# vivansxu/rafiki

Hardware: AMD Instinct MI355X
Metric: images/sec aggregate over concurrent VGG-small 32x32x3 HPO trials (1 trial/GPU) (higher is better)
Workload: dtype fp32; 1 GPU; model=VGG-small 32x32x3 (8 conv3x3+BN+ReLU, 4 maxpool, FC512, FC10), global_batch=256, per_trial_batch=256, parallelism=single trial, 1 GPU, optimizer=SGD nesterov momentum + wd (fused flat-arena kernel), hipgraph=True

## Files before the change

### rafiki_amd/engine/convnet.py

```python
from __future__ import annotations

import math
import os
import warnings
from typing import List, Optional, Sequence

import numpy as np
import torch
import torch.nn.functional as TF

from ..ops import f32 as S
from ..ops import functional as F
from ..ops.graphs import capture as _capture, device_sync as _device_sync
from .flat import FlatAdam, FlatParams, FlatSGD, init_const, init_kaiming

VGG_SMALL_CFG = (64, 64, 'M', 128, 128, 'M', 256, 256, 'M', 512, 512, 'M')
DTYPES = ('fp32', 'bf16')


def default_dtype() -> str:
    d = os.environ.get('RAFIKI_DTYPE', 'fp32').lower()
    d = {'float32': 'fp32', 'f32': 'fp32', 'bfloat16': 'bf16'}.get(d, d)
    if d not in DTYPES:
        raise ValueError('RAFIKI_DTYPE must be one of {}'.format(DTYPES))
# ... 344 lines not shown
                else:
                    d = F.conv_dgrad(dy, fl.wb(name + '.w'))

    def _bn_on_load(self, bi, B, ww):
        if ww is None or bi + 1 >= len(self.blocks):
            return False
        name, cin, cout, pool, hw = self.blocks[bi]
        nxt = self.blocks[bi + 1]
        return (not pool and nxt[1] == cout and nxt[4] == hw and ww.lazy('u4b', bi + 1) is not None
                and S.bn_on_load_ok(B, hw, hw, cout, nxt[2]))

    def _fwd_bwd_gpu_f32(self, x, labels):
        fl = self.flat
        B = x.shape[0]
        accs = self._bn_accumulators()
        if not self._acc_zeroed_by_prologue:
            self._bn_acc_flat.zero_()
        ww = self._wino_train()
        if ww is not None:
            ww.refresh()
        acts, saved, h = [x], [], x
        pros, hpro = [None], None
        for bi, (name, cin, cout, pool, hw) in enumerate(self.blocks):
            wk = ww.conv_sets(bi) if ww is not None else {}
            if not self.bn:
                c = self._block_coeffs(bi)
                y = S.conv_fwd(h, fl.w(name + '.w'), bias=fl.w(name + '.b'),
                               act=F.ACT_NONE if pool else F.ACT_RELU, **wk)
                h = S.bn_eval(y, c[2], c[3], pool=True, act=F.ACT_RELU) if pool else y
                saved.append((y, c))
                acts.append(h)
                continue
            rm, rv = self.running_stats(bi)
            y = S.conv_fwd(h, fl.w(name + '.w'), stats_acc=accs[bi][0], pro=hpro, **wk)
            if self._bn_on_load(bi, B, ww):
                coeffs = S.bn_finalize(y, accs[bi][0], B * hw * hw, fl.w(name + '.gamma'), fl.w(name + '.beta'),
                                       self.bn_eps, rm, rv, self.bn_momentum)
                h, hpro = y, coeffs
            else:
                h, coeffs = S.bn_fwd(y, accs[bi][0], B * hw * hw, fl.w(name + '.gamma'), fl.w(name + '.beta'),
                                     self.bn_eps, rm, rv, self.bn_momentum, pool=pool, act=F.ACT_RELU)
                hpro = None
            saved.append((y, coeffs))
            acts.append(h)
            pros.append(hpro)
        in_saved = None
        if self.input_bn:
            raw = h.reshape(B, 1, 1, self.feat_dim)
            acc_f, acc_b = accs[-1]
            S.col_stats(raw.view(B, self.feat_dim), acc_f)
            rm, rv = self.running_stats('in')
            h, coeffs = S.bn_fwd(raw, acc_f, B, fl.w('in_bn.gamma'), fl.w('in_bn.beta'), self.bn_eps, rm, rv,
                                 self.bn_momentum, pool=False, act=F.ACT_NONE)
            in_saved = (raw, coeffs)
        feat = h.reshape(B, self.feat_dim)
        if self.feature_dropout > 0.0:
            self._drop(feat, -1, self.feature_dropout, forward=True)
        fc_in = [feat]
        z = feat
        for k, (name, di, do, _) in enumerate(self.fcs):
            z = S.linear(z, fl.w(name + '.w'), fl.w(name + '.b'), act=F.ACT_RELU)
            if self.dropout > 0.0:
                self._drop(z, k, self.dropout, forward=True)
            fc_in.append(z)
        dlogits = torch.empty((B, self.ncls_p), dtype=torch.float32, device=self.device)
        k_top = len(self.fcs) - 1
        if self.fused_head and S.head_ok(self.ncls_p, self.d_last):
# ... 26 lines not shown
            else:
                S.softmax_xent(logits, labels, self.num_classes, dlogits=dlogits, loss_sum=self.loss_sum,
                               correct=self.correct, counted=self.seen)
            S.linear_dw(dlogits, fc_in[-1], out=fl.g('out.w'))
            S.colsum(dlogits, fl.g('out.b'))
            d, wname = dlogits, 'out'
        for k in range(k_top, -1, -1):
            name = self.fcs[k][0]
            d = S.linear_dx(d, fl.w(wname + '.w'), gate=fc_in[k + 1])
            if self.dropout > 0.0:
                self._drop(d, k, self.dropout)
            S.linear_dw(d, fc_in[k], out=fl.g(name + '.w'))
            S.colsum(d, fl.g(name + '.b'))
            wname = name
        if not self.blocks and not self.input_bn:
            return
        if wname is not None:
            d = S.linear_dx(d, fl.w(wname + '.w'))
            if self.feature_dropout > 0.0:
                self._drop(d, -1, self.feature_dropout)
        if self.input_bn:
            raw, coeffs = in_saved
            S.bn_bwd(d.view(B, 1, 1, self.feat_dim), raw, coeffs, fl.w('in_bn.gamma'), accs[-1][1], pool=False,
                     act=F.ACT_NONE, dgamma=fl.g('in_bn.gamma'), dbeta=fl.g('in_bn.beta'))
            return
        d = d.view(B, self.feat_hw, self.feat_hw, -1)
        wt = self._conv_wt()
        if wt is not None:
            wt.begin_step()
        reduced = False
        for bi in range(len(self.blocks) - 1, -1, -1):
            name, cin, cout, pool, hw = self.blocks[bi]
            y, coeffs = saved[bi]
            if self.bn:
                dy = S.bn_bwd(d, y, coeffs, fl.w(name + '.gamma'), accs[bi][1], pool=pool, act=F.ACT_RELU,
                              dgamma=fl.g(name + '.gamma'), dbeta=fl.g(name + '.beta'), reduced=reduced)
            else:
                dy = S.bn_bwd(d, y, coeffs, self._ones[:cout], accs[bi][1], pool=pool, act=F.ACT_RELU,
                              dbeta=fl.g(name + '.b'), reduced=reduced, count=float('inf'))
            S.conv_wgrad(dy, acts[bi], out=fl.g(name + '.w').view(cout, -1),
                         xpro=pros[bi] if self.bn else None)
            if bi == 0:
                break
            py, pco = saved[bi - 1]
            pname, pcin, pcout, ppool, phw = self.blocks[bi - 1]
            wl = wt.lazy(bi - 1)
            dk = dict(ww.conv_sets(bi, dgrad=True) if ww is not None else {}, cin=cin)
            if not ppool:
                d = S.conv_dgrad(dy, wl, bnb=(py, pco, accs[bi - 1][1]), **dk)
                reduced = True
            elif phw == 2 * hw and not (hw & (hw - 1)):
                d = S.conv_dgrad(dy, wl, bnp=(py, pco, accs[bi - 1][1]), **dk)
                reduced = True
            else:
                d = S.conv_dgrad(dy, wl, **dk)
                reduced = False
        if ww is not None:
            ww.end_step()

    def _wino_train(self):
        if not (self.f32 and S.WINO and self.blocks and self.device.type == 'cuda'):
            return None
        ww = getattr(self, '_ww', None)
        if ww is None:
            fl = self.flat
            ww = self._ww = S.WinoWeights(fl.master, [fl.w(b[0] + '.w') for b in self.blocks],
# ... 635 lines not shown
```

### rafiki_amd/ops/_lib.py

```python
from __future__ import annotations

import ctypes as C
import os
import threading
from pathlib import Path

_NATIVE = Path(__file__).resolve().parent.parent / "_native"
KERNEL_LIB = Path(os.environ["RAFIKI_KERNEL_LIB"]) if os.environ.get("RAFIKI_KERNEL_LIB") else \
    _NATIVE / "librafiki_kernels.so"

_lock = threading.Lock()
_lib = None

vp, i32, i64, f32, f64 = C.c_void_p, C.c_int, C.c_longlong, C.c_float, C.c_double
u32p = C.POINTER(C.c_uint)

_SIGS = {
    "rk_igemm": [i32, i32, i32, vp, vp, vp, vp, vp, vp, i32, i32, i32, i32, i32, i32, i32, i32, i32, i32,
                 i32, i32, i64, i32, f32, f32, i64, i64, vp],
    "rk_hconv": [i32, i32, vp, vp, vp, vp, vp, vp, i32, i32, i32, i32, i32, i32, i32, i32, f32, f32, i64, i64, i32,
                 vp],
    "rk_hconv_wgrad": [vp, vp, vp, i32, i32, i32, i32, i32, i32, i64, i64, vp],
    "rk_bn_bwd_reduce_acc": [vp, vp, vp, vp, vp, i32, i32, i32, i32, i32, i32, i32, i32, f32, vp],
    "rk_bn_bwd_apply_acc": [vp, vp, vp, vp, i32, f64, vp, vp, vp, vp, i32, vp, i32, i32, i32, i32, i32, i32, f32, vp],
# ... 31 lines not shown
    "rk_nonfinite": [vp, i64, vp, vp],
    "rk_reduce_slabs": [vp, i32, i64, vp, i32, f32, vp],
    "rk_colsum": [vp, i32, i32, i32, vp, i32, vp],
    "rk_ensemble_mean": [vp, i32, i64, vp, vp, vp],
    "rk_cast_f32_bf16": [vp, vp, i64, vp],
    "rk_pack_nhwc": [vp, i32, i32, i32, i32, i32, i32, f32, f32, vp, vp],
    "rk_philox": [vp, i64, i32, i32, f32, f32, C.c_ulonglong, C.c_uint, vp, vp],
    "rk_lrelu_pixelnorm": [vp, vp, vp, i32, i32, f32, f32, vp, vp],
    "rk_mbstd": [i32, vp, vp, vp, i32, i32, i32, i32, i32, i32, vp, vp, vp, vp],
    "rk_colsum_part": [vp, i32, i32, i32, i32, vp, vp],
    "rk_lstm_fwd": [vp, vp, i32, i32, i32, vp, vp, vp, vp],
    "rk_lstm_bwd": [vp, i32, i32, i32, vp, vp, vp, vp, vp],
    "rk_lstm_fwd32": [vp, vp, i32, i32, i32, vp, vp, vp, vp],
    "rk_lstm_bwd32": [vp, i32, i32, i32, vp, vp, vp, vp, vp],
    "rk_wino_weights": [vp, vp, vp, i32, i32, vp],
    "rk_wino_conv_grp": [vp, vp, vp, vp, vp, i32, vp, i32, i32, i32, i32, i32, i32, i32, i32, i64, i64, i64, i64, vp],
    "rk_wino_wgrad": [vp, vp, vp, i32, i32, i32, i32, i32, i32, i32, vp],
    "rk_wino4_weights": [vp, vp, vp, i32, i32, vp],
    "rk_wino4b_weights": [vp, vp, vp, i32, i32, vp],
    "rk_wino4_conv_grp": [vp, vp, vp, vp, vp, i32, vp, i32, i32, i32, i32, i32, i32, i32, i32, i64, i64, i64, i64, vp,
                          vp],
    "rk_wino4_wgrad": [vp, vp, vp, i32, i32, i32, i32, i32, i32, i32, i32, vp, vp],
    "rk_wino4_pt_transform": [vp, vp, vp, vp, i32, i32, i32, i32, i32, vp, vp],
    "rk_wino4_pt_output": [vp, vp, i32, i32, i32, i32, i64, vp],
    "rk_wino4_pt_input": [vp, vp, i32, i32, i32, i32, vp, vp],
    "rk_wino4_pt_conv_out": [vp, vp, vp, vp, i32, vp, i32, i32, i32, i32, i32, i32, i64, i32, f32, vp],
    "rk_wino2s_conv_grp": [vp, vp, vp, vp, vp, i32, vp, i32, i32, i32, i32, i32, i32, i32, i32, i64, i64, i64, i64, vp],
    "rk_sgemm": [i32, i32, i32, vp, vp, vp, vp, vp, i32, vp, i32, i32, i32, i32, i32, i32, i32, i32, i32, i32, i32,
                 i64, i32, f32, f32, i64, i64, vp],
    "rk_bnf_fwd": [vp, vp, i32, f64, vp, vp, f32, vp, vp, f32, vp, vp, vp, vp, i32, i32, i32, i32, i32, i32, f32, vp],
    "rk_bnf_bwd_reduce": [vp, vp, vp, vp, i32, i32, i32, i32, i32, i32, i32, i32, f32, vp],
    "rk_bnf_bwd_apply": [vp, vp, vp, vp, i32, f64, vp, vp, vp, i32, vp, i32, i32, i32, i32, i32, i32, f32, vp],
    "rk_bnf_colstats": [vp, vp, i32, i32, vp, vp],
    "rk_swt": [vp, vp, vp, i32, vp, vp],
    "rk_colsum_f32": [vp, i32, i32, i32, vp, i32, i32, vp],
    "rk_lrelu_gate_f32": [vp, vp, vp, i64, f32, vp],
    "rk_lrelu_gate_colsum_f32": [vp, vp, vp, i32, i32, f32, vp, i32, vp],
    "rk_wgan_loss_fwd": [vp, i32, i32, vp, i32, f32, f32, f32, vp, vp, vp, vp],
    "rk_wgan_mix": [vp, vp, vp, vp, vp, i32, i32, vp],
    "rk_wgan_loss_bwd": [vp, vp, i32, i32, vp, i32, f32, f32, f32, vp, vp, vp, vp],
    "rk_sreduce_epi": [vp, i32, i32, i32, vp, i32, f32, f32, vp, i32, vp, i32, i32, vp],
    "rk_sgemm_grp": [i32, i32, i32, vp, vp, vp, vp] + [i32] * 10 + [i32, i64, i32, f32, f32, i64, i64, i32, i64, i64,
                                                                     i64, i64, vp],
    "rk_bnf_eval_grp": [vp, vp, vp, vp, i32, i32, i32, i32, i32, i32, i32, f32, vp],
    "rk_pack_nhwc_f32": [vp, i32, i32, i32, i32, i32, i32, f32, f32, vp, vp, i32, vp],
    "rk_softmax_xent_f32": [vp, i32, vp, i32, i32, i32, f32, vp, i32, vp, vp, vp, vp, vp],
    "rk_softmax_xent_f32_soft": [vp, i32, vp, vp, vp, f32, i32, i32, i32, f32, vp, i32, vp, vp, vp, vp],
    "rk_sgemm_g": [i32, i32, i32, vp, vp, vp, vp] + [i32] * 14 + [u32p, u32p, C.c_uint, i32, i64, i32, i64, i32, f32,
                                                                 f32, i64, i64, vp],
    "rk_resample2x": [i32, i32, vp, vp, i32, i32, i32, i32, f32, vp],
    "rk_s2t_weights": [vp, vp, i32, i32, vp],
    "rk_box_weights": [i32, vp, vp, i32, i32, f32, vp],
    "rk_wflip_t": [vp, vp, i32, i32, i32, vp],
    "rk_mbstd_f32": [i32, vp, vp, vp, i32, i32, i32, i32, i32, i32, vp, vp, vp, vp],
    "rk_lrelu_pixelnorm_f32": [vp, vp, vp, i32, i32, f32, f32, vp, vp],
    "rk_embedding_fwd": [vp, vp, vp, i32, i32, i32, vp],
    "rk_embedding_bwd": [vp, vp, vp, i32, i32, i32, i32, vp, i64, vp],
    "rk_tag_embed_fwd": [vp, vp, vp, vp, i32, i32, i32, f32, C.c_ulonglong, i32, vp, vp],
    "rk_tag_embed_bwd": [vp, vp, vp, vp, vp, vp, vp, i32, i32, i32, vp],
    "rk_tag_transpose": [vp, vp, i32, i32, i32, vp],
    "rk_tag_add": [vp, vp, vp, i64, vp],
    "rk_softmax_xent_f32s": [vp, i32, vp, i32, i32, i32, vp, vp, i32, vp, vp],
    "rk_head_fwd_bwd": [vp, i32, i32, vp, vp, i32, vp, i32, f32, vp, vp, i32, vp, vp, vp, vp],
    "rk_head_fwd_bwd_soft": [vp, i32, i32, vp, vp, i32, vp, vp, vp, f32, i32, f32, vp, vp, i32, vp, vp, vp, vp],
    "rk_head_dw": [vp, vp, vp, i32, i32, i32, vp, vp, vp, vp],
    "rk_dropout": [vp, i64, i32, f32, C.c_ulonglong, C.c_uint, vp, vp, vp],
# ... 66 lines not shown
```

### rafiki_amd/ops/autotune.py

```python
from __future__ import annotations

import fcntl
import hashlib
import json
import os
import sys
import threading

import torch

from .graphs import LOCK as _GRAPH_LOCK, capture as _capture

_lock = threading.Lock()
_cache = {}
_loaded = False
_disk_mtime = [None]
stats = {'tuned': 0, 'seconds': 0.0, 'candidates': 0, 'loaded': 0, 'reloads': 0}
_last_note = [0.0]
ENABLED = os.environ.get('RAFIKI_AUTOTUNE', '1') != '0'
REPS = 3
PASSES = 2
SHIPPED_DIR = os.path.join(os.path.dirname(os.path.dirname(os.path.abspath(__file__))), 'tune')
_ident = {}

# ... 7 lines not shown
            _ident['arch'] = os.environ.get('RAFIKI_OFFLOAD_ARCH', 'gfx950')
    return _ident['arch']


_SRC_DIR = os.path.join(os.path.dirname(os.path.dirname(os.path.dirname(os.path.abspath(__file__)))), 'csrc',
                        'kernels')


def lib_hash() -> str:
    if 'lib' not in _ident:
        h = hashlib.sha1()
        try:
            srcs = sorted(f for f in os.listdir(_SRC_DIR) if f.endswith(('.hip', '.h')))
        except OSError:
            srcs = []
        try:
            if srcs:
                for f in srcs:
                    h.update(f.encode())
                    with open(os.path.join(_SRC_DIR, f), 'rb') as fh:
                        h.update(fh.read())
                _ident['lib'] = 's' + h.hexdigest()[:11]
            else:
                from ._lib import loaded_path as lib_path
                with open(lib_path(), 'rb') as f:
                    for chunk in iter(lambda: f.read(1 << 20), b''):
                        h.update(chunk)
                _ident['lib'] = h.hexdigest()[:12]
        except OSError:
            _ident['lib'] = 'nolib'
    return _ident['lib']


_CAND_SWITCHES = ('RAFIKI_X6', 'RAFIKI_PT_MAX_HW', 'RAFIKI_WINOGRAD', 'RAFIKI_WINOGRAD4')


def db_name() -> str:
    tag = ','.join('{}={}'.format(k, os.environ[k]) for k in _CAND_SWITCHES if k in os.environ)
    suffix = '-' + hashlib.sha1(tag.encode()).hexdigest()[:8] if tag else ''
    return '{}-{}{}.json'.format(_arch(), lib_hash(), suffix)


def _path():
    p = os.environ.get('RAFIKI_TUNE_CACHE')
    if p is not None and p.lower() in ('off', '0', 'none', ''):
        return ''
    if p:
        return p
    from ..config import get_config
    return os.path.join(get_config().workdir, 'tune', db_name())


def _tup(v):
    return tuple(_tup(x) for x in v) if isinstance(v, list) else v


def _read(path):
    try:
        with open(path) as f:
            return {_tup(json.loads(k)): _tup(v) for k, v in json.load(f).items()}
    except (OSError, ValueError):
        return {}


def _load():
    global _loaded
    if _loaded:
# ... 177 lines not shown
```

### rafiki_amd/ops/f32.py

```python
from __future__ import annotations

import os
from functools import partial
from typing import NamedTuple, Optional

import torch

from . import _lib, autotune
from .functional import ACT_LRELU, ACT_NONE, ACT_RELU, _check_soft, bn_slots, cdiv, dropout_

KIND_CONV, KIND_WGRAD, KIND_DENSE, KIND_DENSE_DX, KIND_DENSE_DW = 0, 2, 3, 4, 5
F_RELU, F_BIAS, F_STATS, F_GATE, F_ACCUM, F_LRELU, F_BNB, F_BNP = 1, 2, 4, 8, 16, 32, 512, 1024
TILES = [(128, 128), (128, 64), (64, 128), (64, 64), (256, 64), (256, 128), (128, 256), (64, 256),
         (64, 64), (128, 64), (64, 128)]
_NST3 = (0, 1, 2, 3, 4, 7)
_FEW_WAVE = (8, 9, 10)
NUM_CU = 256
X6 = 16
USE_X6 = os.environ.get('RAFIKI_X6', '1') != '0'


def tile_dims(t: int):
    return TILES[t & 15]

# ... 134 lines not shown
    *_set_pair('u4b', 'ut4b', 'wino4b', 3, 'rk_wino4b_weights', lambda r, c: wino4b_numel(r, c),
               lambda flat, r, c: flat, 1, lambda f4, hw, r, c: _f4_map(f4, hw) and c % 8 == 0, padded=True),
)
KIND = {k.name: k for k in SET_KINDS}
SET_KWARGS = tuple(k.kwarg for k in SET_KINDS if not k.dgrad)


def conv_sets(lazy, dgrad=False):
    return {k.kwarg: lazy(k.name) for k in SET_KINDS if k.dgrad == bool(dgrad)}


def _set_dims(k, Cout, Cin):
    return (Cin, Cout) if k.dgrad else (Cout, Cin)


def wino_set(kind: str, w: torch.Tensor) -> torch.Tensor:
    k = KIND[kind]
    Cout = w.shape[0]
    Cin = w.numel() // (9 * Cout)
    rows, cols = _set_dims(k, Cout, Cin)
    flat = (torch.zeros if k.padded else torch.empty)(k.size(rows, cols), device=w.device, dtype=torch.float32)
    out = k.view(flat, rows, cols)
    _lib.call(k.entry, _p(w), None if k.dgrad else _p(out), _p(out) if k.dgrad else None, Cout, Cin, _s())
    return out


def _offered(families, sets, taps, H, W, C, N, need):
    on = [sets[f.weights] is not None and taps == 9 and not (need & ~f.also) and f.offer(H, W, C, N)
          for f in families]
    return on, [c for f, o in zip(families, on) if o for c in f.cfgs]


def _sets_key(sets, on):
    w2, w4, w4b, pt, ptx = on
    return (('lazy' if callable(sets[0]) else w2, 'lazy' if callable(sets[1]) else w4, pt,
             'lazy' if callable(sets[2]) else ptx) + (('b', 'lazy' if callable(sets[3]) else True),) * w4b)


def _run_route(r, x, sets, out, cfg, epi):
    u = sets[r.weights]
    r.kernel(x, u() if callable(u) else u, out=out, **SLOTS[r.slots](r, cfg), **epi)


def conv_fwd(x: torch.Tensor, w: torch.Tensor, *, taps: int = 9, stats_acc=None, bias=None, act=ACT_NONE,
             slope=0.2, out=None, wino=None, wino4=None, wino4p=None, wino4b=None, pro=None):
    _check(x, 'conv_fwd x')
    Nb, H, W, Cin = x.shape
    Cout = w.shape[0]
    M, K = Nb * H * W, taps * Cin
    assert w.numel() == Cout * K, (w.shape, taps, Cin)
    if out is None:
        out = torch.empty((Nb, H, W, Cout), device=x.device, dtype=torch.float32)
    flags = (F_STATS if stats_acc is not None else 0) | (F_BIAS if bias is not None else 0)
    flags |= F_RELU if act == ACT_RELU else F_LRELU if act == ACT_LRELU else 0
    sets = (wino, wino4, wino4p, wino4b)
    epi = dict(bias=bias, stats=stats_acc, relu=act == ACT_RELU)
    need = 0
    if act == ACT_LRELU:
        need, epi['lrelu'] = E_LRELU if stats_acc is None else E_DIRECT, slope
    if pro is not None:
        assert bias is None and act == ACT_NONE and pro.shape == (4, Cin)
        need, epi['pro'], cands = E_PRO, pro, []
    else:
        cands = _cands(M, Cout, splittable=stats_acc is None and Cout % 4 == 0, K=K, big=Cin % 32 == 0)
    on, fused = _offered(CONV_FAMILIES, sets, taps, H, W, Cin, Cout, need)
    cands += fused
    if not cands:
        raise ValueError('conv_fwd(pro=...): no normalise-on-load kernel for this shape (see bn_on_load_ok)')

    def run(cfg):
        r = CONV_ROUTES.get(cfg[0])
        if r is not None:
            _run_route(r, x, sets, out, cfg, epi)
            return
        tile, nst, s = cfg
        if s == 1:
            sgemm(KIND_CONV, x, w, out, M, Cout, K, Cin, K, Cout, tile=tile, nst=nst, bias=bias, stats=stats_acc,
                  H=H, W=W, C=Cin, taps=taps, flags=flags, slope=slope)
            return
        slab = torch.empty((s, M, Cout), device=x.device, dtype=torch.float32)
        sgemm(KIND_CONV, x, w, slab, M, Cout, K, Cin, K, Cout, tile=tile, nst=nst, splits=s, slab_stride=M * Cout,
              H=H, W=W, C=Cin, taps=taps)
        sreduce_epi(slab, M, Cout, out.view(M, Cout), bias=bias, act=act, slope=slope)
    cfg = _pick(('sf', M, Cout, K, H, W, Cin, taps, flags) + _sets_key(sets, on)
                + (('pro',) if pro is not None else ()), cands, run)
    if stats_acc is not None and autotune.can_tune():
        stats_acc.zero_()
    run(cfg)
    return out


def conv_dgrad(dy: torch.Tensor, wt, *, taps: int = 9, out=None, gate=None, bnb=None, bnp=None,
               wino=None, wino4=None, cin=None, wino4p=None, wino4b=None):
    _check(dy, 'conv_dgrad dy')
    Nb, H, W, Cout = dy.shape
    Cin = cin if callable(wt) else wt.shape[0]
    M, K = Nb * H * W, taps * Cout
    assert callable(wt) or wt.numel() == Cin * K
    if out is None:
        out = torch.empty((Nb, H, W, Cin), device=dy.device, dtype=torch.float32)
    flags, bias, stats = 0, None, None
    if bnb is not None:
        y, coeffs, stats = bnb
        assert y.shape == out.shape and stats.dtype == torch.float64 and stats.shape[-1] == Cin
        gate, bias, flags = y, coeffs[2:4].reshape(-1), F_BNB
    elif bnp is not None:
        y, coeffs, stats = bnp
        assert y.shape == (Nb, 2 * H, 2 * W, Cin) and stats.dtype == torch.float64
        assert not (H & (H - 1)) and not (W & (W - 1)), 'pooled BN fusion needs power-of-two maps'
        gate, bias, flags = y, coeffs[2:4].reshape(-1), F_BNP
    elif gate is not None:
        flags = F_GATE
    sets = (wino, wino4, wino4p, wino4b)
    epi = dict(bnb=bnb, bnp=bnp)
    on, fused = _offered(CONV_FAMILIES, sets, taps, H, W, Cout, Cin, E_DIRECT if flags & F_GATE else 0)
    cands = _cands(M, Cin, big=Cout % 32 == 0) + fused

    def run(cfg):
        r = CONV_ROUTES.get(cfg[0])
        if r is not None:
            _run_route(r, dy, sets, out, cfg, epi)
            return
        sgemm(KIND_CONV, dy, wt() if callable(wt) else wt, out, M, Cin, K, Cout, K, Cin, tile=cfg[0], nst=cfg[1],
              bias=bias, stats=stats, gate=gate, H=H, W=W, C=Cout, taps=taps, flags=flags)
    cfg = _pick(('sd', M, Cin, K, H, W, Cout, taps, flags) + _sets_key(sets, on), cands, run)
    if stats is not None and autotune.can_tune():
        stats.zero_()
    run(cfg)
    return out


def _lead_with_split(cands, M, N):
    split = [c for c in cands if c[2] > 1]
    if not split:
        return cands
    return [max(split, key=lambda c: min(cdiv(M, tile_dims(c[0])[0]) * cdiv(N, tile_dims(c[0])[1]) * c[2],
                                         2 * NUM_CU))] + cands


def conv_wgrad(dy: torch.Tensor, x: torch.Tensor, *, taps: int = 9, out=None, accumulate=False, xpro=None):
    _check(dy, 'conv_wgrad dy')
    _check(x, 'conv_wgrad x')
    Nb, H, W, Cout = dy.shape
    Cin = x.shape[-1]
    M, N, K = Cout, taps * Cin, Nb * H * W
    if out is None:
# ... 423 lines not shown
        tps = cdiv(cdiv(nt, s), 8) * 8
        s_eff = cdiv(nt, tps)
        if tps < 64 or base * s_eff > 4096 or (s_eff > 1 and s_eff * 9 * Cout * Cin * 4 > (256 << 20)):
            continue
        if base * s_eff < 128 and s != 1:
            continue
        c = (WINO_WGRAD, 0, s_eff)
        if c not in out:
            out.append(c)
    return out


def wino_wgrad(dy: torch.Tensor, x: torch.Tensor, out: torch.Tensor, *, splits=1, accumulate=False):
    _check(dy, 'wino_wgrad dy')
    _check(x, 'wino_wgrad x')
    Nb, H, W, Cout = dy.shape
    Cin = x.shape[-1]
    assert x.shape[:3] == dy.shape[:3] and out.numel() == Cout * 9 * Cin and out.is_contiguous()
    if splits == 1:
        _lib.call("rk_wino_wgrad", _p(dy), _p(x), _p(out), Nb, H, W, Cout, Cin, 1, int(bool(accumulate)), _s())
        return out
    slab = torch.empty((splits, Cout, 9 * Cin), device=dy.device, dtype=torch.float32)
    _lib.call("rk_wino_wgrad", _p(dy), _p(x), _p(slab), Nb, H, W, Cout, Cin, int(splits), 0, _s())
    reduce_slabs(slab, out.view(Cout, 9 * Cin), accumulate=accumulate)
    return out


def wino_conv_grp(x, u, *, out=None, bias=None, relu=False, variant=0, pool=False):
    H, W = x.shape[-3:-1]
    assert not pool or (bias is not None and relu and variant >= 2 and H % 2 == 0 and W % 2 == 0)
    return _grp_conv(*_wino2_entry(variant), 16, x, u, out, bias, relu, pool)


class Route(NamedTuple):
    id: int
    name: str
    slots: str
    kernel: object
    offer: object
    cfgs: tuple = ()
    family: str = ''
    weights: int = 0
    variant: int = 0
    also: int = 0
    grp: object = None
    pool: bool = False


E_LRELU, E_PRO, E_DIRECT = 1, 2, 4
SLOTS = {
    'fixed: 0, 1': lambda r, cfg: {'variant': r.variant},
    '0, K splits': lambda r, cfg: {'splits': cfg[2]},
    'kernel variant, K splits': lambda r, cfg: {'variant': cfg[1], 'splits': cfg[2]},
    'sgemm tile code, ring depth': lambda r, cfg: {'tile': cfg[1], 'nst': cfg[2]},
    'x6p code, K splits': lambda r, cfg: dict(zip(('tile', 'nst'), x6p_unpack(cfg[1])), splits=cfg[2]),
}
_SGEMM, _X6P = 'sgemm tile code, ring depth', 'x6p code, K splits'


def _fused(id, name, variant, kernel, **kw):
    return Route(id, name, 'fixed: 0, 1', kernel, cfgs=((id, 0, 1),), variant=variant, **kw)


_F2 = dict(family='f2', weights=0, offer=lambda H, W, C, N: wino_ok(H, W, C), grp=wino_conv_grp)
_F4 = dict(family='f4', weights=1, offer=lambda H, W, C, N: wino4_ok(H, W, C), grp=wino4_conv_grp, pool=True)
_F4B = dict(family='f4b', weights=3, offer=_F4['offer'], also=E_PRO)
WINO4_PT, WINO4_PTX = -14, -15
WINO_WGRAD, WINO4_WGRAD, WINO4_WGRAD_PT, WINO4_WGRAD_PTX = -3, -7, -13, -16
WINO4_PTX_CFGS = tuple((WINO4_PTX, x6p_pack(t, n), s) for t, n, s in _XP_CFGS) if USE_X6P else ()
CONV_ROUTES = {r.id: r for r in (
    _fused(-1, 'F(2x2) 4-wave 64x32', 0, wino_conv, **_F2),
    _fused(-2, 'F(2x2) 8-wave 64x64', 1, wino_conv, **_F2),
    _fused(-8, 'F(2x2) 4-wave 32x32', 2, wino_conv, pool=True, **_F2),
    _fused(-9, 'F(2x2) 2-wave 16x32', 3, wino_conv, pool=True, **_F2),
    _fused(-10, 'F(2x2) 8-wave 64x32', 4, wino_conv, pool=True, **_F2),
    _fused(-12, 'F(2x2) 8-wave 64x32 two-stage', 5, wino_conv, pool=True, **_F2),
    _fused(-5, 'F(4x4) 8-wave 64 tiles x 32 channels', 0, wino4_conv, **_F4),
    _fused(-6, 'F(4x4) 4-wave 32 x 32', 1, wino4_conv, **_F4),
    _fused(-17, 'F(4x4) blocked, 8-wave tile of -5', 3, wino4_conv, **_F4B),
    _fused(-18, 'F(4x4) blocked, 4-wave tile of -6', 4, wino4_conv, **_F4B),
    _fused(-19, 'F(4x4) blocked, warp-specialised (4 compute + 4 loader waves, two LDS stages)', 5, wino4_conv, **_F4B),
    Route(WINO4_PT, 'F(4x4) pre-transformed', _SGEMM, wino4_conv_pt, cfgs=_pt_cfgs(WINO4_PT), family='pt',
          weights=1, offer=lambda H, W, C, N: wino4_ok(H, W, C) and wino4_pt_ok(H, W, C, N), also=E_LRELU | E_PRO),
    Route(WINO4_PTX, 'F(4x4) pre-transformed, X6 planes', _X6P, wino4_conv_pt, cfgs=WINO4_PTX_CFGS,
          family='ptx', weights=2, offer=lambda H, W, C, N: wino4_ptx_ok(H, W, C, N), also=E_LRELU | E_PRO),
)}
WGRAD_ROUTES = {r.id: r for r in (
    Route(WINO_WGRAD, 'F(2x2) weight gradient', '0, K splits', wino_wgrad, _wino_wgrad_cands),
    Route(WINO4_WGRAD, 'F(4x4) weight gradient', 'kernel variant, K splits', wino4_wgrad, _wino4_wgrad_cands,
          also=E_PRO),
    Route(WINO4_WGRAD_PT, 'F(4x4) pre-transformed weight gradient', _SGEMM, wino4_wgrad_pt, _wino4_pt_cands,
          also=E_PRO),
    Route(WINO4_WGRAD_PTX, 'F(4x4) pre-transformed weight gradient, X6 planes', _X6P,
          partial(wino4_wgrad_pt, planes=True), _wino4_ptx_wgrad_cands),
)}


def _family(name):
    rows = [r for r in CONV_ROUTES.values() if r.family == name]
    shared = [(r.weights, r.offer, r.also, r.grp) for r in rows]
    assert shared.count(shared[0]) == len(rows), name
    return rows[0]._replace(name=name, cfgs=tuple(c for r in rows for c in r.cfgs))


CONV_FAMILIES = tuple(_family(n) for n in ('f2', 'f4', 'f4b', 'pt', 'ptx'))
GRP_FAMILIES = CONV_FAMILIES[:2]


class WinoWeights:

    KINDS = tuple(k.name for k in SET_KINDS)

    def __init__(self, arena: torch.Tensor, weights, dgrad=True, f4=None, hw=None):
        self.arena = arena
        self.weights = list(weights)
        self.dgrad = dgrad
        f4 = WINO4 if f4 is None else f4
        self._layers, self._sets, off = [], {}, 0
        for l, w in enumerate(self.weights):
            Cout = w.shape[0]
            Cin = w.numel() // (9 * Cout)
            so = (w.data_ptr() - arena.data_ptr()) // 4
            assert 0 <= so and so + w.numel() <= arena.numel() and w.is_contiguous()
            self._layers.append((so, Cout, Cin))
            for k in SET_KINDS:
                rows, cols = _set_dims(k, Cout, Cin)
                if (dgrad or not k.dgrad) and k.offered(f4, None if hw is None else hw[l], rows, cols):
                    self._sets[(k.name, l)] = (off, k.size(rows, cols))
                    off += k.size(rows, cols)
        self.buf = torch.zeros(max(off, 1), dtype=torch.float32, device=arena.device)
        self._tables = {}
        self.live = frozenset(self._sets)
        self._fresh = set()
        self._used = set()
        self._prepare(self.live)

    def _prepare(self, live):
        if live not in self._tables:
# ... 645 lines not shown
```

Measured before the change: 140,400 images/s.

## Add direct stem conv kernels with fused BN-backward weight gradient

Adds specialised HIP kernels for the first conv layer, whose input has only a few real channels (padded to 4 or 8): a direct forward conv that accumulates BN statistics, and a fused BN-backward plus weight-gradient kernel. Both are registered as autotuned routes alongside the existing Winograd and GEMM paths. The goal is to avoid wasting GEMM or Winograd work on padded input channels and to drop the separate bn_bwd pass and its dy tensor for the stem layer. The fused backward adds a partial-slab buffer and a reduction step, and both paths depend on the autotuner picking them.

```diff
diff --git a/csrc/kernels/stem.hip b/csrc/kernels/stem.hip
--- /dev/null
+++ b/csrc/kernels/stem.hip
@@ -0,0 +1,252 @@
+#include "common.h"
+#include <algorithm>
+
+namespace {
+
+RK_DEV int idiv(int a, int d, int log2d) { return log2d >= 0 ? a >> log2d : a / d; }
+
+RK_DEV float act_d(float z, int act, float slope) {
+  return act == 1 ? (z > 0.f ? 1.f : 0.f) : act == 2 ? (z > 0.f ? 1.f : slope) : 1.f;
+}
+
+constexpr int WAVES = 4;
+constexpr int UNR = 8;
+constexpr int UNR_F = 4;
+
+struct Geo {
+  int H, W, lH, lW, cin_p;
+};
+
+RK_DEV void stage_x(const float* __restrict__ x, float* xs, int q0, int nq, int npix, int cin_p) {
+  const int per = cin_p >> 2, lper = per >> 1;
+  for (int i = threadIdx.x; i < nq * per; i += 256) {
+    const int q = q0 + (i >> lper);
+    f32x4 v = {0.f, 0.f, 0.f, 0.f};
+    if ((unsigned)q < (unsigned)npix) v = *(const f32x4*)(x + (long long)q * cin_p + (i & (per - 1)) * 4);
+    *(f32x4*)(xs + i * 4) = v;
+  }
+  __syncthreads();
+}
+
+template <int CR>
+RK_DEV void lane_tap(int lane, const Geo& g, int& dh, int& dw, int& off) {
+  const int t = lane / CR, ci = lane - t * CR;
+  dw = t % 3 - 1;
+  off = ((t / 3 - 1) * g.W + dw) * g.cin_p + ci;
+  dh = lane < 9 * CR ? t / 3 - 1 : g.H;
+}
+
+template <int CR>
+RK_DEV void load_patch(const float* xs, int p, int q0, const Geo& g, int dh, int dw, int off, float (&xv)[9][CR]) {
+  const int t = idiv(p, g.W, g.lW);
+  const int w = p - t * g.W;
+  const int h = t - idiv(t, g.H, g.lH) * g.H;
+  float val = 0.f;
+  if ((unsigned)(h + dh) < (unsigned)g.H && (unsigned)(w + dw) < (unsigned)g.W) val = xs[(p - q0) * g.cin_p + off];
+#pragma unroll
+  for (int k = 0; k < 9 * CR; ++k)
+    xv[k / CR][k % CR] = __builtin_bit_cast(float, __builtin_amdgcn_readlane(__builtin_bit_cast(int, val), k));
+}
+
+template <int CR>
+__global__ __launch_bounds__(256) void stem_wgrad_bn_kernel(
+    const float* __restrict__ dz, const float* __restrict__ y, const float* __restrict__ coeffs,
+    const double* __restrict__ slots, int SL, double count, const float* __restrict__ gamma,
+    float* __restrict__ dgamma, float* __restrict__ dbeta, const float* __restrict__ x, float* __restrict__ part,
+    int npix, int ppb, int nq, Geo g, int Co, int act, float slope) {
+  constexpr int NA = 9 * CR, LD = NA | 1;
+  extern __shared__ __attribute__((aligned(16))) float smem[];
+  const int tid = threadIdx.x, lane = tid & 63;
+  const int wave = __builtin_amdgcn_readfirstlane(tid >> 6);
+  const int c0 = blockIdx.y * 64, c = c0 + lane;
+  const int p0 = min(npix, blockIdx.x * ppb), p1 = min(npix, p0 + ppb), q0 = p0 - g.W - 1;
+  stage_x(x, smem, q0, nq, npix, g.cin_p);
+  float a, b, cc;
+  {
+    double s0 = 0.0, s1 = 0.0;
+    for (int l = 0; l < SL; ++l) {
+      s0 += slots[(long long)l * 2 * Co + c];
+      s1 += slots[(long long)l * 2 * Co + Co + c];
+    }
+    const double mean = coeffs[c], rstd = coeffs[Co + c];
+    const double T = rstd * (s1 - mean * s0);
+    const double A = (double)gamma[c] * rstd;
+    const double B = -A * rstd * T / count;
+    a = (float)A;
+    b = (float)B;
+    cc = (float)(-A * s0 / count - B * mean);
+    if (blockIdx.x == 0 && wave == 0) {
+      if (dgamma) dgamma[c] = (float)T;
+      if (dbeta) dbeta[c] = (float)s0;
+    }
+  }
+  const float sc = coeffs[2 * Co + c], sh = coeffs[3 * Co + c];
+  int dh, dw, off;
+  lane_tap<CR>(lane, g, dh, dw, off);
+  float acc[9][CR];
+#pragma unroll
+  for (int t = 0; t < 9; ++t)
+#pragma unroll
+    for (int ci = 0; ci < CR; ++ci) acc[t][ci] = 0.f;
+  for (int pb = p0 + wave; pb < p1; pb += WAVES * UNR) {
+    float d[UNR], v[UNR];
+#pragma unroll
+    for (int u = 0; u < UNR; ++u) {
+      const int p = pb + u * WAVES;
+      d[u] = v[u] = 0.f;
+      if (p < p1) {
+        d[u] = dz[(long long)p * Co + c];
+        v[u] = y[(long long)p * Co + c];
+      }
+    }
+#pragma unroll
+    for (int u = 0; u < UNR; ++u) {
+      const int p = pb + u * WAVES;
+      if (p >= p1) break;
+      float xv[9][CR];
+      load_patch<CR>(smem, p, q0, g, dh, dw, off, xv);
+      const float o = a * (d[u] * act_d(v[u] * sc + sh, act, slope)) + b * v[u] + cc;
+#pragma unroll
+      for (int t = 0; t < 9; ++t)
+#pragma unroll
+        for (int ci = 0; ci < CR; ++ci) acc[t][ci] += o * xv[t][ci];
+    }
+  }
+  __syncthreads();
+  float* red = smem;
+#pragma unroll
+  for (int t = 0; t < 9; ++t)
+#pragma unroll
+    for (int ci = 0; ci < CR; ++ci) red[(wave * 64 + lane) * LD + t * CR + ci] = acc[t][ci];
+  __syncthreads();
+  const int row = 9 * g.cin_p;
+  float* dst = part + ((long long)blockIdx.x * Co + c0) * row;
+  for (int i = tid; i < 64 * row; i += 256) {
+    const int co = i / row, r = i - co * row;
+    const int t = r / g.cin_p, ci = r - t * g.cin_p;
+    float s = 0.f;
+    if (ci < CR) {
+      const float* rk = red + co * LD + t * CR + ci;
+      s = (rk[0] + rk[64 * LD]) + (rk[2 * 64 * LD] + rk[3 * 64 * LD]);
+    }
+    dst[i] = s;
+  }
+}
+
+template <int CR>
+__global__ __launch_bounds__(256) void stem_conv_fwd_kernel(const float* __restrict__ x, const float* __restrict__ w,
+                                                            float* __restrict__ out, double* __restrict__ stats,
+                                                            int slotMask, int npix, int ppb, int nq, Geo g, int Co) {
+  extern __shared__ __attribute__((aligned(16))) float smem[];
+  const int tid = threadIdx.x, lane = tid & 63;
+  const int wave = __builtin_amdgcn_readfirstlane(tid >> 6);
+  const int c = blockIdx.y * 64 + lane;
+  const int p0 = min(npix, blockIdx.x * ppb), p1 = min(npix, p0 + ppb), q0 = p0 - g.W - 1;
+  stage_x(x, smem, q0, nq, npix, g.cin_p);
+  float wv[9][CR];
+#pragma unroll
+  for (int t = 0; t < 9; ++t)
+#pragma unroll
+    for (int ci = 0; ci < CR; ++ci) wv[t][ci] = w[((long long)c * 9 + t) * g.cin_p + ci];
+  int dh, dw, off;
+  lane_tap<CR>(lane, g, dh, dw, off);
+  float s = 0.f, ss = 0.f;
+  for (int pb = p0 + wave; pb < p1; pb += WAVES * UNR_F) {
+#pragma unroll
+    for (int u = 0; u < UNR_F; ++u) {
+      const int p = pb + u * WAVES;
+      if (p >= p1) break;
+      float xv[9][CR];
+      load_patch<CR>(smem, p, q0, g, dh, dw, off, xv);
+      float o = 0.f;
+#pragma unroll
+      for (int t = 0; t < 9; ++t)
+#pragma unroll
+        for (int ci = 0; ci < CR; ++ci) o += xv[t][ci] * wv[t][ci];
+      out[(long long)p * Co + c] = o;
+      s += o;
+      ss += o * o;
+    }
+  }
+  if (!stats) return;
+  __syncthreads();
+  float* red = smem;
+  red[wave * 64 + lane] = s;
+  red[(WAVES + wave) * 64 + lane] = ss;
+  __syncthreads();
+  if (wave == 0) {
+    const float ts = (red[lane] + red[64 + lane]) + (red[128 + lane] + red[192 + lane]);
+    const float tss = (red[256 + lane] + red[320 + lane]) + (red[384 + lane] + red[448 + lane]);
+    double* sl = stats + (long long)(blockIdx.x & slotMask) * 2 * Co;
+    unsafeAtomicAdd(sl + c, (double)ts);
+    unsafeAtomicAdd(sl + Co + c, (double)tss);
+  }
+}
+
+bool stem_shape_ok(int Nb, int H, int W, int Co, int cin_p, int cin_real, int blocks) {
+  if (Nb < 1 || H < 1 || W < 1 || blocks < 1 || blocks > 65535) return false;
+  if (Co < 64 || Co % 64 || (cin_p != 4 && cin_p != 8) || cin_real < 1 || cin_real > 4) return false;
+  return (long long)Nb * H * W * Co < (1ll << 31);
+}
+
+Geo stem_geo(int H, int W, int cin_p) { return Geo{H, W, rk_log2(H), rk_log2(W), cin_p}; }
+
+bool aligned16(const void* p) { return !(reinterpret_cast<uintptr_t>(p) & 15); }
+
+constexpr long long STEM_MAX_LDS = 64 << 10;
+
+}
+
+extern "C" int rk_stem_wgrad_bn(const float* dz, const float* y, const float* coeffs, const double* slots, int SL,
+                                double count, const float* gamma, float* dgamma, float* dbeta, const float* x,
+                                float* part, int blocks, int Nb, int H, int W, int Co, int cin_p, int cin_real,
+                                int act, float slope, void* stream) {
+  if (!stem_shape_ok(Nb, H, W, Co, cin_p, cin_real, blocks) || SL < 1) return RK_EUNSUPPORTED;
+  if (!dz || !y || !coeffs || !slots || !gamma || !x || !part) return RK_EBADARG;
+  if (!aligned16(x)) return RK_EUNSUPPORTED;
+  const int npix = Nb * H * W, ppb = rk_cdiv(npix, blocks);
+  const long long nq = (long long)ppb + 2 * W + 2;
+  const long long lds = std::max(nq * cin_p * 4, (long long)WAVES * 64 * ((9 * cin_real) | 1) * 4);
+  if (lds > STEM_MAX_LDS) return RK_EUNSUPPORTED;
+  const dim3 grid(blocks, Co / 64);
+  const Geo g = stem_geo(H, W, cin_p);
+  hipStream_t st = (hipStream_t)stream;
+#define STEM_WGRAD(CR)                                                                                           \
+  hipLaunchKernelGGL(stem_wgrad_bn_kernel<CR>, grid, dim3(256), (size_t)lds, st, dz, y, coeffs, slots, SL, count, \
+                     gamma, dgamma, dbeta, x, part, npix, ppb, (int)nq, g, Co, act, slope)
+  switch (cin_real) {
+    case 1: STEM_WGRAD(1); break;
+    case 2: STEM_WGRAD(2); break;
+    case 3: STEM_WGRAD(3); break;
+    default: STEM_WGRAD(4); break;
+  }
+#undef STEM_WGRAD
+  RK_LAUNCH_CHECK();
+  return RK_OK;
+}
+
+extern "C" int rk_stem_conv_fwd(const float* x, const float* w, float* out, double* stats, int slot_mask, int blocks,
+                                int Nb, int H, int W, int Co, int cin_p, int cin_real, void* stream) {
+  if (!stem_shape_ok(Nb, H, W, Co, cin_p, cin_real, blocks) || (slot_mask & (slot_mask + 1))) return RK_EUNSUPPORTED;
+  if (!x || !w || !out) return RK_EBADARG;
+  if (!aligned16(x)) return RK_EUNSUPPORTED;
+  const int npix = Nb * H * W, ppb = rk_cdiv(npix, blocks);
+  const long long nq = (long long)ppb + 2 * W + 2;
+  const long long lds = std::max(nq * cin_p * 4, (long long)2 * WAVES * 64 * 4);
+  if (lds > STEM_MAX_LDS) return RK_EUNSUPPORTED;
+  const dim3 grid(blocks, Co / 64);
+  const Geo g = stem_geo(H, W, cin_p);
+  hipStream_t st = (hipStream_t)stream;
+#define STEM_FWD(CR)                                                                                               \
+  hipLaunchKernelGGL(stem_conv_fwd_kernel<CR>, grid, dim3(256), (size_t)lds, st, x, w, out, stats, slot_mask, npix, \
+                     ppb, (int)nq, g, Co)
+  switch (cin_real) {
+    case 1: STEM_FWD(1); break;
+    case 2: STEM_FWD(2); break;
+    case 3: STEM_FWD(3); break;
+    default: STEM_FWD(4); break;
+  }
+#undef STEM_FWD
+  RK_LAUNCH_CHECK();
+  return RK_OK;
+}
diff --git a/rafiki_amd/engine/convnet.py b/rafiki_amd/engine/convnet.py
--- a/rafiki_amd/engine/convnet.py
+++ b/rafiki_amd/engine/convnet.py
@@ -400,7 +400,8 @@
                 acts.append(h)
                 continue
             rm, rv = self.running_stats(bi)
-            y = S.conv_fwd(h, fl.w(name + '.w'), stats_acc=accs[bi][0], pro=hpro, **wk)
+            y = S.conv_fwd(h, fl.w(name + '.w'), stats_acc=accs[bi][0], pro=hpro,
+                           cin_real=self.in_channels if bi == 0 else None, **wk)
             if self._bn_on_load(bi, B, ww):
                 coeffs = S.bn_finalize(y, accs[bi][0], B * hw * hw, fl.w(name + '.gamma'), fl.w(name + '.beta'),
                                        self.bn_eps, rm, rv, self.bn_momentum)
@@ -493,6 +494,11 @@
         for bi in range(len(self.blocks) - 1, -1, -1):
             name, cin, cout, pool, hw = self.blocks[bi]
             y, coeffs = saved[bi]
+            if bi == 0 and self.bn and not pool and reduced and S.STEM_DIRECT:
+                S.bn_bwd_wgrad(d, y, coeffs, fl.w(name + '.gamma'), accs[bi][1], acts[bi],
+                               out=fl.g(name + '.w').view(cout, -1), cin_real=self.in_channels, act=F.ACT_RELU,
+                               dgamma=fl.g(name + '.gamma'), dbeta=fl.g(name + '.beta'))
+                break
             if self.bn:
                 dy = S.bn_bwd(d, y, coeffs, fl.w(name + '.gamma'), accs[bi][1], pool=pool, act=F.ACT_RELU,
                               dgamma=fl.g(name + '.gamma'), dbeta=fl.g(name + '.beta'), reduced=reduced)
diff --git a/rafiki_amd/ops/_lib.py b/rafiki_amd/ops/_lib.py
--- a/rafiki_amd/ops/_lib.py
+++ b/rafiki_amd/ops/_lib.py
@@ -87,6 +87,8 @@
     "rk_bnf_bwd_reduce": [vp, vp, vp, vp, i32, i32, i32, i32, i32, i32, i32, i32, f32, vp],
     "rk_bnf_bwd_apply": [vp, vp, vp, vp, i32, f64, vp, vp, vp, i32, vp, i32, i32, i32, i32, i32, i32, f32, vp],
     "rk_bnf_colstats": [vp, vp, i32, i32, vp, vp],
+    "rk_stem_conv_fwd": [vp, vp, vp, vp, i32, i32, i32, i32, i32, i32, i32, i32, vp],
+    "rk_stem_wgrad_bn": [vp, vp, vp, vp, i32, f64, vp, vp, vp, vp, vp, i32, i32, i32, i32, i32, i32, i32, i32, f32, vp],
     "rk_swt": [vp, vp, vp, i32, vp, vp],
     "rk_colsum_f32": [vp, i32, i32, i32, vp, i32, i32, vp],
     "rk_lrelu_gate_f32": [vp, vp, vp, i64, f32, vp],
diff --git a/rafiki_amd/ops/autotune.py b/rafiki_amd/ops/autotune.py
--- a/rafiki_amd/ops/autotune.py
+++ b/rafiki_amd/ops/autotune.py
@@ -63,7 +63,7 @@
     return _ident['lib']
 
 
-_CAND_SWITCHES = ('RAFIKI_X6', 'RAFIKI_PT_MAX_HW', 'RAFIKI_WINOGRAD', 'RAFIKI_WINOGRAD4')
+_CAND_SWITCHES = ('RAFIKI_X6', 'RAFIKI_PT_MAX_HW', 'RAFIKI_WINOGRAD', 'RAFIKI_WINOGRAD4', 'RAFIKI_STEM_DIRECT')
 
 
 def db_name() -> str:
diff --git a/rafiki_amd/ops/f32.py b/rafiki_amd/ops/f32.py
--- a/rafiki_amd/ops/f32.py
+++ b/rafiki_amd/ops/f32.py
@@ -190,9 +190,10 @@
 
 
 def _sets_key(sets, on):
-    w2, w4, w4b, pt, ptx = on
+    w2, w4, w4b, pt, ptx, stem = on
     return (('lazy' if callable(sets[0]) else w2, 'lazy' if callable(sets[1]) else w4, pt,
-             'lazy' if callable(sets[2]) else ptx) + (('b', 'lazy' if callable(sets[3]) else True),) * w4b)
+             'lazy' if callable(sets[2]) else ptx) + (('b', 'lazy' if callable(sets[3]) else True),) * w4b
+            + (('stem',) + STEM_FWD_BLOCKS,) * stem)
 
 
 def _run_route(r, x, sets, out, cfg, epi):
@@ -201,7 +202,7 @@
 
 
 def conv_fwd(x: torch.Tensor, w: torch.Tensor, *, taps: int = 9, stats_acc=None, bias=None, act=ACT_NONE,
-             slope=0.2, out=None, wino=None, wino4=None, wino4p=None, wino4b=None, pro=None):
+             slope=0.2, out=None, wino=None, wino4=None, wino4p=None, wino4b=None, pro=None, cin_real=None):
     _check(x, 'conv_fwd x')
     Nb, H, W, Cin = x.shape
     Cout = w.shape[0]
@@ -211,7 +212,8 @@
         out = torch.empty((Nb, H, W, Cout), device=x.device, dtype=torch.float32)
     flags = (F_STATS if stats_acc is not None else 0) | (F_BIAS if bias is not None else 0)
     flags |= F_RELU if act == ACT_RELU else F_LRELU if act == ACT_LRELU else 0
-    sets = (wino, wino4, wino4p, wino4b)
+    stem = (w, cin_real) if flags == F_STATS and pro is None and stem_ok(Cout, Cin, cin_real) else None
+    sets = (wino, wino4, wino4p, wino4b, stem)
     epi = dict(bias=bias, stats=stats_acc, relu=act == ACT_RELU)
     need = 0
     if act == ACT_LRELU:
@@ -269,7 +271,7 @@
         gate, bias, flags = y, coeffs[2:4].reshape(-1), F_BNP
     elif gate is not None:
         flags = F_GATE
-    sets = (wino, wino4, wino4p, wino4b)
+    sets = (wino, wino4, wino4p, wino4b, None)
     epi = dict(bnb=bnb, bnp=bnp)
     on, fused = _offered(CONV_FAMILIES, sets, taps, H, W, Cout, Cin, E_DIRECT if flags & F_GATE else 0)
     cands = _cands(M, Cin, big=Cout % 32 == 0) + fused
@@ -759,6 +761,74 @@
     return _grp_conv(*_wino2_entry(variant), 16, x, u, out, bias, relu, pool)
 
 
+STEM_DIRECT = os.environ.get('RAFIKI_STEM_DIRECT', '1') != '0'
+STEM_FWD, STEM_WGRAD_BN = -22, -23
+STEM_FWD_BLOCKS = (1024, 2048, 4096)
+STEM_WGRAD_BLOCKS = (256, 512, 1024)
+
+
+def stem_ok(Cout: int, cin_p: int, cin_real) -> bool:
+    return bool(STEM_DIRECT and Cout >= 64 and Cout % 64 == 0 and cin_p in (4, 8) and cin_real is not None
+                and 1 <= cin_real <= min(4, cin_p))
+
+
+def stem_conv_fwd(x: torch.Tensor, w: torch.Tensor, *, cin_real: int, out=None, stats=None, blocks=2048, bias=None,
+                  relu=False):
+    _check(x, 'stem_conv_fwd x')
+    _check(w, 'stem_conv_fwd w')
+    assert bias is None and not relu, 'the direct stem conv carries BN statistics only'
+    Nb, H, W, Cin = x.shape
+    Cout = w.shape[0]
+    assert w.numel() == Cout * 9 * Cin
+    assert stats is None or (stats.dtype == torch.float64 and stats.is_contiguous() and stats.shape[1:] == (2, Cout))
+    if out is None:
+        out = torch.empty((Nb, H, W, Cout), device=x.device, dtype=torch.float32)
+    _lib.call("rk_stem_conv_fwd", _p(x), _p(w), _p(out), _p(stats), _slots_flags(stats), int(blocks), Nb, H, W, Cout,
+              Cin, int(cin_real), _s())
+    return out
+
+
+def stem_wgrad_bn(dz, y, coeffs, gamma, acc, x, out, *, cin_real: int, blocks=512, act=ACT_RELU, slope=0.2,
+                  dgamma=None, dbeta=None, accumulate=False, count=None):
+    _check(dz, 'stem_wgrad_bn dz')
+    _check(y, 'stem_wgrad_bn y')
+    _check(x, 'stem_wgrad_bn x')
+    Nb, H, W, Cout = y.shape
+    Cin = x.shape[-1]
+    assert dz.shape == y.shape and x.shape[:3] == y.shape[:3] and coeffs.shape == (4, Cout)
+    assert out.numel() == Cout * 9 * Cin and out.is_contiguous()
+    assert acc.dtype == torch.float64 and acc.is_contiguous() and acc.shape[1:] == (2, Cout)
+    part = torch.empty((int(blocks), Cout, 9 * Cin), device=y.device, dtype=torch.float32)
+    _lib.call("rk_stem_wgrad_bn", _p(dz), _p(y), _p(coeffs), _p(acc), acc.shape[0],
+              float(Nb * H * W) if count is None else float(count), _p(gamma), _p(dgamma), _p(dbeta), _p(x), _p(part),
+              int(blocks), Nb, H, W, Cout, Cin, int(cin_real), int(act), float(slope), _s())
+    reduce_slabs(part, out.view(Cout, 9 * Cin), accumulate=accumulate)
+    return out
+
+
+def bn_bwd_wgrad(dz, y, coeffs, gamma, acc, x, *, out, cin_real=None, act=ACT_RELU, slope=0.2, dgamma=None,
+                 dbeta=None, accumulate=False):
+    Nb, H, W, Cout = y.shape
+    Cin = x.shape[-1]
+
+    def run(cfg):
+        if cfg[0] == STEM_WGRAD_BN:
+            stem_wgrad_bn(dz, y, coeffs, gamma, acc, x, out, cin_real=cin_real, blocks=cfg[1], act=act, slope=slope,
+                          dgamma=dgamma, dbeta=dbeta, accumulate=accumulate)
+            return
+        dy = bn_bwd(dz, y, coeffs, gamma, acc, act=act, slope=slope, dgamma=dgamma, dbeta=dbeta, reduced=True)
+        conv_wgrad(dy, x, out=out, accumulate=accumulate)
+    two_calls = (0, 0, 1)
+    if not stem_ok(Cout, Cin, cin_real):
+        run(two_calls)
+        return out
+    cands = [two_calls] + [(STEM_WGRAD_BN, b, 1) for b in STEM_WGRAD_BLOCKS]
+    cfg = _pick(('sbw', Nb, H, W, Cout, Cin, int(cin_real), int(act), bool(accumulate), 'two calls', 'stem')
+                + STEM_WGRAD_BLOCKS, cands, run, protect=(out,) if accumulate else ())
+    run(cfg)
+    return out
+
+
 class Route(NamedTuple):
     id: int
     name: str
@@ -781,6 +851,7 @@
     'kernel variant, K splits': lambda r, cfg: {'variant': cfg[1], 'splits': cfg[2]},
     'sgemm tile code, ring depth': lambda r, cfg: {'tile': cfg[1], 'nst': cfg[2]},
     'x6p code, K splits': lambda r, cfg: dict(zip(('tile', 'nst'), x6p_unpack(cfg[1])), splits=cfg[2]),
+    'pixel blocks, 1': lambda r, cfg: {'blocks': cfg[1]},
 }
 _SGEMM, _X6P = 'sgemm tile code, ring depth', 'x6p code, K splits'
 
@@ -811,6 +882,10 @@
           weights=1, offer=lambda H, W, C, N: wino4_ok(H, W, C) and wino4_pt_ok(H, W, C, N), also=E_LRELU | E_PRO),
     Route(WINO4_PTX, 'F(4x4) pre-transformed, X6 planes', _X6P, wino4_conv_pt, cfgs=WINO4_PTX_CFGS,
           family='ptx', weights=2, offer=lambda H, W, C, N: wino4_ptx_ok(H, W, C, N), also=E_LRELU | E_PRO),
+    Route(STEM_FWD, 'direct stem conv, <= 4 real input channels', 'pixel blocks, 1',
+          lambda x, u, **kw: stem_conv_fwd(x, u[0], cin_real=u[1], **kw),
+          cfgs=tuple((STEM_FWD, b, 1) for b in STEM_FWD_BLOCKS), family='stem', weights=4,
+          offer=lambda H, W, C, N: stem_ok(N, C, 1)),
 )}
 WGRAD_ROUTES = {r.id: r for r in (
     Route(WINO_WGRAD, 'F(2x2) weight gradient', '0, K splits', wino_wgrad, _wino_wgrad_cands),
@@ -830,7 +905,7 @@
     return rows[0]._replace(name=name, cfgs=tuple(c for r in rows for c in r.cfgs))
 
 
-CONV_FAMILIES = tuple(_family(n) for n in ('f2', 'f4', 'f4b', 'pt', 'ptx'))
+CONV_FAMILIES = tuple(_family(n) for n in ('f2', 'f4', 'f4b', 'pt', 'ptx', 'stem'))
 GRP_FAMILIES = CONV_FAMILIES[:2]
 
 
```

After: 141,600 images/s (median of 6 runs). Within noise of the previous version (+0.9%).
